# CrystalSixone/VLN-MAGIC

Hardware: AMD Instinct MI355X
Metric: trajectory-steps/sec (whole node), MAGIC-S R2R pretrain (higher is better)
Workload: dtype bf16

## Files before the change

### vln-magic_amd/csrc/encbwd.hip

```cpp
#include "enc_common.hpp"
#include <cstdlib>
#include <cstring>


template <typename Hh> struct RbwSegT {
  int M, kt;
  const Hh* dqkv_n; const Hh* WqkvT_n; const Hh* dao_n;
  const Hh* dfo_in; const Hh* dfod_in;
  const Hh* y2; const float* rstd2; const float* g2; const float* b2; float* dg2; float* db2;
  const Hh* z; const Hh* W2T; const Hh* W1T;
  const Hh* y1; const float* rstd1; const float* g1; const float* b1; float* dg1; float* db1;
  const Hh* WoT;
  Hh *dfo, *dfod, *dz, *daod, *dao, *dctx;
  unsigned site_out, site_ao;
  int mode, N, ntile, ldp;
  const Hh* qkv_a; const Hh* P_a; const Hh* o_a; const Hh* dctx_a; const float* dP_init;
  Hh* dqkv_out;
  unsigned site_attn, pad_;
  const float* dist; float* dsprel_w; float* dsprel_b;
};
template <typename Hh> struct RbwParamsT { RbwSegT<Hh> seg[2]; int nseg, blocks0; float p_hidden; int pad1; const unsigned* seed; float p_attn, scale; };
typedef RbwParamsT<bf16> RbwParams; typedef RbwSegT<bf16> RbwSeg;
#define F(f) ABI_VIEW(RbwSeg, magic_rowbwd_seg, f)
F(M) F(kt) F(dqkv_n) F(WqkvT_n) F(dao_n) F(dfo_in) F(dfod_in) F(y2) F(rstd2) F(g2) F(b2) F(dg2) F(db2) F(z) F(W2T) F(W1T) F(y1) F(rstd1) F(g1) F(b1)
F(dg1) F(db1) F(WoT) F(dfo) F(dfod) F(dz) F(daod) F(dao) F(dctx) F(site_out) F(site_ao) F(mode) F(N) F(ntile) F(ldp) F(qkv_a) F(P_a) F(o_a) F(dctx_a)
F(dP_init) F(dqkv_out) F(site_attn) F(pad_) F(dist) F(dsprel_w) F(dsprel_b)
#undef F
#define F(f) ABI_VIEW(RbwParams, magic_rowbwd_params, f)
F(seg) F(nseg) F(blocks0) F(p_hidden) F(pad1) F(seed) F(p_attn) F(scale)
#undef F

__device__ __forceinline__ float dgelu_fast(float x) {
  const float ax = fabsf(x) * 0.70710678118654752f;
  const float t = __builtin_amdgcn_rcpf(1.0f + 0.3275911f * ax);
  const float poly = t * (0.254829592f + t * (-0.284496736f + t * (1.421413741f + t * (-1.453152027f + t * 1.061405429f))));
  const float e = __expf(-ax * ax);
  const float erf_abs = 1.0f - poly * e;
  const float cdf = 0.5f * (1.0f + (x < 0.f ? -erf_abs : erf_abs));
  return cdf + x * 0.39894228040143268f * e;
}

template <typename Hh> __device__ __forceinline__ void load_rows_img(Hh* s, int pitch, const Hh* g, long long ldg, int rows, int cols, int nvalid, int tid) {
  const int cpr = cols / 8;
  for (int id = tid; id < rows * cpr; id += NWAVE * 64) {
    const int r = id / cpr, c = (id % cpr) * 8;
    h16x8<Hh> v;
#pragma unroll
    for (int e = 0; e < 8; ++e) v[e] = (Hh)0.0f;
    if (r < nvalid) v = *(const h16x8<Hh>*)(g + (long long)r * ldg + c);
    *(h16x8<Hh>*)(s + r * pitch + c) = v;
  }
}

template <int NRT, typename Hh>
__device__ __forceinline__ void ln_bwd_rows(f32x4 (&acc)[NRT], const Hh* sY, const float* rstd_g, const float gm, const float bt, float* dgamma,
                                            float* dbeta, float* red, Hh* sSum, Hh* sDense, const int m0, const int M, const DropState& ds,
                                            const int w, const int lane, const int part_blk = -1) {
  constexpr int RB_ROWS = NRT * 16;
  const int g = lane >> 4, c16 = lane & 15, col = w * 16 + c16;
  const float ig = gm != 0.f ? 1.f / gm : 0.f;
  float xh[NRT][4], s1[NRT][4], s2[NRT][4];
  float pg = 0.f, pb = 0.f;
#pragma unroll
  for (int i = 0; i < NRT; ++i)
#pragma unroll
    for (int r = 0; r < 4; ++r) {
      const int rr = i * 16 + 4 * g + r;
      const bool live = m0 + rr < M;
      const float v = live ? acc[i][r] : 0.f;
      const float x = live ? (to_f(sY[rr * XS + col]) - bt) * ig : 0.f;
      pg += v * x; pb += v;
      const float ga = v * gm;
      acc[i][r] = ga; xh[i][r] = x;
      s1[i][r] = row16_sum(ga); s2[i][r] = row16_sum(ga * x);
    }
  if (dgamma) {
    pg += __shfl_xor(pg, 16, 64); pg += __shfl_xor(pg, 32, 64);
    pb += __shfl_xor(pb, 16, 64); pb += __shfl_xor(pb, 32, 64);
    if (g == 0) {
      if (part_blk >= 0) { dgamma[(long long)part_blk * EH + col] = pg; dbeta[(long long)part_blk * EH + col] = pb; }
      else { atomicAdd(dgamma + col, pg); atomicAdd(dbeta + col, pb); }
    }
  }
  if (c16 == 0) {
#pragma unroll
    for (int i = 0; i < NRT; ++i)
#pragma unroll
      for (int r = 0; r < 4; ++r) { red[w * RB_ROWS + i * 16 + 4 * g + r] = s1[i][r]; red[(NWAVE + w) * RB_ROWS + i * 16 + 4 * g + r] = s2[i][r]; }
  }
  __syncthreads();
#pragma unroll
  for (int i = 0; i < NRT; ++i)
#pragma unroll
    for (int r = 0; r < 4; ++r) {
      const int rr = i * 16 + 4 * g + r;
      float t1 = 0.f, t2 = 0.f;
#pragma unroll
      for (int ww = 0; ww < NWAVE; ++ww) { t1 += red[ww * RB_ROWS + rr]; t2 += red[(NWAVE + ww) * RB_ROWS + rr]; }
      const float m1 = t1 * (1.0f / EH), m2 = t2 * (1.0f / EH);
      const float rs = (m0 + rr < M) ? rstd_g[m0 + rr] : 0.f;
      const float d = rs * (acc[i][r] - m1 - xh[i][r] * m2);
      sSum[rr * XS + col] = from_f<Hh>(d);
      sDense[rr * XS + col] = from_f<Hh>(ds.on ? d * drop_mul(ds, (unsigned)((m0 + rr) * EH + col)) : d);
    }
}

#ifdef RBW_TIMING
__device__ long long rbw_ticks[32];
#define RBW_MARK(i) do { if (blockIdx.x == 0 && threadIdx.x == 0) rbw_ticks[i] = wall_clock64(); } while (0)
#else
#define RBW_MARK(i)
#endif
#define AT_DS 72
#define AT_PS 104
#define AT_ROWS 96
static inline size_t attn_stage_lds() { return (size_t)(3 * AT_ROWS * AT_DS + 3 * 16 * AT_PS) * 2 + AT_ROWS * sizeof(float); }
template <typename Hh, bool DIST>
__device__ __forceinline__ void attn_tile_stage(const RbwSegT<Hh>& sg, const RbwParamsT<Hh>& p, const int b, const int ti, const int nv,
                                                Hh* sDq, unsigned char* scratch, const int tid) {
  typedef h16x4<Hh> v4;
  const int lane = tid & 63, w = __builtin_amdgcn_readfirstlane(tid >> 6), g = lane >> 4, c16 = lane & 15;
  const int N = sg.N, NT = sg.ntile, NK32 = (N + 31) / 32 * 32, ldp = sg.ldp;
  Hh* sQ = (Hh*)scratch;
  Hh* sK = sQ + AT_ROWS * AT_DS;
  Hh* sdO = sK + AT_ROWS * AT_DS;
  Hh* sdS = sdO + AT_ROWS * AT_DS;
  Hh* sdST = sdS + 16 * AT_PS;
  Hh* sPT = sdST + 16 * AT_PS;
  float* sRs = (float*)(sPT + 16 * AT_PS);
  const long long row0 = (long long)b * N;
  DropDesc dd;
  dd.seed = p.seed; dd.site = sg.site_attn; dd.p = p.p_attn;
  const DropState ds = drop_init(dd);
  h16x8<Hh> zero8;
#pragma unroll
  for (int e = 0; e < 8; ++e) zero8[e] = (Hh)0.0f;
  for (int id = tid; id < 3 * 16 * AT_PS / 8; id += NWAVE * 64) *(h16x8<Hh>*)(sdS + id * 8) = zero8;
  constexpr int RIT = (AT_ROWS * 8 + NWAVE * 64 - 1) / (NWAVE * 64);
  static_assert(RIT == 2, "image-row load mapping");
  h16x8<Hh> rq[RIT], rk[RIT], ro[RIT], rO[RIT];
  auto img_issue = [&](const int h) {
#pragma unroll
    for (int it = 0; it < RIT; ++it) {
      const int id = tid + it * NWAVE * 64, r = id >> 3, c = (id & 7) * 8;
      rq[it] = zero8; rk[it] = zero8; ro[it] = zero8; rO[it] = zero8;
      if (r < N) {
        const Hh* base = sg.qkv_a + (row0 + r) * (3 * EH) + h * EHD + c;
        rq[it] = *(const h16x8<Hh>*)base;
        rk[it] = *(const h16x8<Hh>*)(base + EH);
        ro[it] = *(const h16x8<Hh>*)(sg.dctx_a + (row0 + r) * EH + h * EHD + c);
        rO[it] = *(const h16x8<Hh>*)(sg.o_a + (row0 + r) * EH + h * EHD + c);
      }
    }
  };
  auto img_store = [&](const int h) {
#pragma unroll
    for (int it = 0; it < RIT; ++it) {
      const int id = tid + it * NWAVE * 64, r = id >> 3, c = (id & 7) * 8;
      if (r < NK32) {
        *(h16x8<Hh>*)(sQ + r * AT_DS + c) = rq[it];
        *(h16x8<Hh>*)(sK + r * AT_DS + c) = rk[it];
        *(h16x8<Hh>*)(sdO + r * AT_DS + c) = ro[it];
      }
      float s = 0.f;
#pragma unroll
      for (int e = 0; e < 8; ++e) s += to_f(ro[it][e]) * to_f(rO[it][e]);
      if (DIST && sg.dP_init && r < N) {
        const long long prow = ((long long)b * ENH + h) * N + r;
        for (int c8 = (id & 7) * 8; c8 < ldp; c8 += 64) {
          const h16x8<Hh> pv = *(const h16x8<Hh>*)(sg.P_a + prow * ldp + c8);
          const f32x4 i0 = *(const f32x4*)(sg.dP_init + prow * ldp + c8), i1 = *(const f32x4*)(sg.dP_init + prow * ldp + c8 + 4);
#pragma unroll
          for (int e = 0; e < 8; ++e) {
            const int key = c8 + e;
            if (key < N) {
              const float m = ds.on ? drop_mul(ds, (unsigned)(prow * N + key)) : 1.f;
              s += to_f(pv[e]) * m * (e < 4 ? i0[e & 3] : i1[e & 3]);
            }
          }
        }
      }
      s += dpp_mov<DPP_QUAD_XOR1>(s);
      s += dpp_mov<DPP_QUAD_XOR2>(s);
      s += dpp_mov<DPP_ROW_HALF_MIRROR>(s);
      if ((id & 7) == 0 && r < NK32) sRs[r] = s;
    }
  };
  constexpr int AJ = (2 * (AT_ROWS / 16) + NWAVE - 1) / NWAVE;
  h16x8<Hh> av[AJ][EHD / 32];
  v4 ap[AJ];
  f32x4 ai[DIST ? AJ : 1];
  auto vp_issue = [&](const int h) {
#pragma unroll
    for (int jj = 0; jj < AJ; ++jj) {
      const int job = w + NWAVE * jj;
      const bool asq = job < NT;
      const int t = asq ? job : job - NT;
      const int ktile = asq ? t : ti, qtile = asq ? ti : t;
      const int vkey = ktile * 16 + c16, q = qtile * 16 + c16, key0 = ktile * 16 + 4 * g;
      const long long prow = ((long long)b * ENH + h) * N + q;
#pragma unroll
      for (int ks = 0; ks < EHD / 32; ++ks) {
        av[jj][ks] = zero8;
        if (job < 2 * NT && vkey < N) av[jj][ks] = *(const h16x8<Hh>*)(sg.qkv_a + (row0 + vkey) * (3 * EH) + 2 * EH + h * EHD + ks * 32 + 8 * g);
      }
#pragma unroll
      for (int r = 0; r < 4; ++r) ap[jj][r] = (Hh)0.0f;
      if constexpr (DIST) ai[jj] = (f32x4){0.f, 0.f, 0.f, 0.f};
      if (job < 2 * NT && q < N) {
        if (key0 < ldp) ap[jj] = *(const v4*)(sg.P_a + prow * ldp + key0);
        if constexpr (DIST) {
          if (sg.dP_init && key0 < N) ai[jj] = *(const f32x4*)(sg.dP_init + prow * ldp + key0);
        }
      }
    }
  };
  float a0 = 0.f, a1 = 0.f;
  RBW_MARK(16);
  img_issue(0);
  vp_issue(0);
  for (int h = 0; h < ENH; ++h) {
    img_store(h);
    __syncthreads();
    RBW_MARK(17 + 3 * h);
    if (h + 1 < ENH) img_issue(h + 1);
#pragma unroll
    for (int jj = 0; jj < AJ; ++jj) {
      const int job = w + NWAVE * jj;
      if (job < 2 * NT) {
        const bool asq = job < NT;
        const int t = asq ? job : job - NT;
        const int ktile = asq ? t : ti, qtile = asq ? ti : t;
        f32x4 acc = (f32x4){0.f, 0.f, 0.f, 0.f};
#pragma unroll
        for (int ks = 0; ks < EHD / 32; ++ks) acc = mfma16(av[jj][ks], frag_kc(sdO, AT_DS, qtile * 16, ks * 32, lane), acc);
        const int q = qtile * 16 + c16, key0 = ktile * 16 + 4 * g;
        const bool qok = q < N;
        const long long prow = ((long long)b * ENH + h) * N + q;
        const float rsq = sRs[q];
        v4 o4, pm4;
#pragma unroll
        for (int r = 0; r < 4; ++r) {
          const int key = key0 + r;
          const bool ok = qok && key < N;
          float d = acc[r];
          if constexpr (DIST) d += ok ? ai[jj][r] : 0.f;
          const float pp = to_f(ap[jj][r]);
          float pm = pp;
          if (ds.on) {
            const float m = ok ? drop_mul(ds, (unsigned)(prow * N + key)) : 0.f;
            d *= m; pm = pp * m;
          }
          const float dsu = pp * (d - rsq);
          o4[r] = from_f<Hh>(dsu * p.scale);
          pm4[r] = from_f<Hh>(pm);
          if constexpr (DIST) {
            if (sg.dist && asq && ok) { a0 += dsu * sg.dist[((long long)b * N + q) * N + key]; a1 += dsu; }
          }
        }
        if (asq) *(v4*)(sdS + c16 * AT_PS + key0) = o4;
        else {
#pragma unroll
          for (int r = 0; r < 4; ++r) { sdST[(4 * g + r) * AT_PS + q] = o4[r]; sPT[(4 * g + r) * AT_PS + q] = pm4[r]; }
        }
      }
    }
    if (h + 1 < ENH) vp_issue(h + 1);
    __syncthreads();
    RBW_MARK(18 + 3 * h);
    for (int job = w; job < 12; job += NWAVE) {
      const int prod = job >> 2, jd = job & 3;
      const Hh* A = prod == 0 ? sdS : (prod == 1 ? sdST : sPT);
      const Hh* Bm = prod == 0 ? sK : (prod == 1 ? sQ : sdO);
      f32x4 acc = (f32x4){0.f, 0.f, 0.f, 0.f};
      for (int ks = 0; ks < NK32 / 32; ++ks) acc = mfma16(frag_kc(A, AT_PS, 0, ks * 32, lane), frag_oc(Bm, AT_DS, jd * 16, ks * 32, lane), acc);
      const int col = prod * EH + h * EHD + jd * 16 + c16;
#pragma unroll
      for (int r = 0; r < 4; ++r) sDq[(4 * g + r) * QS + col] = from_f<Hh>(acc[r]);
    }
    __syncthreads();
    RBW_MARK(19 + 3 * h);
  }
  copy_out(sDq, QS, sg.dqkv_out + (row0 + ti * 16) * (3 * EH), 3 * EH, nv, 3 * EH, tid);
  if (DIST && sg.dist) {
    a0 = wave_sum(a0); a1 = wave_sum(a1);
    if (lane == 0) { sRs[w] = a0; sRs[NWAVE + w] = a1; }
    __syncthreads();
    if (tid == 0) {
      float s0 = 0.f, s1 = 0.f;
#pragma unroll
      for (int i = 0; i < NWAVE; ++i) { s0 += sRs[i]; s1 += sRs[NWAVE + i]; }
      atomicAdd(sg.dsprel_w, s0);
      atomicAdd(sg.dsprel_b, s1);
    }
    __syncthreads();
  }
  RBW_MARK(23);
}

template <int NRT, typename Hh, int ATT = 0>
__device__ __forceinline__ void rowbwd_body(const RbwParamsT<Hh>& p, unsigned char* rb_smem) {
  constexpr int RB_ROWS = NRT * 16;
  constexpr bool DEEP = NRT >= 4;
  static_assert(!ATT || NRT == 1, "the attention stage works on 16-row tiles of one sample");
  int blk = blockIdx.x, sidx = 0;
  if (blk >= p.blocks0) { blk -= p.blocks0; sidx = 1; }
  const RbwSegT<Hh>& sg = p.seg[sidx];
  const int mode = ATT ? sg.mode : 0;
  Hh* sZ = (Hh*)rb_smem;
  Hh* sY2 = sZ + RB_ROWS * GS;
  Hh* sR = sY2 + RB_ROWS * XS;
  Hh* sFo = sR + RB_ROWS * XS;
  Hh* sD = sFo + RB_ROWS * XS;
  Hh* sY1 = sD + RB_ROWS * XS;
  Hh* sAo = sR;
  float* red = (float*)(sY1 + RB_ROWS * XS);
  const int tid = threadIdx.x, lane = tid & 63, w = __builtin_amdgcn_readfirstlane(tid >> 6), g = lane >> 4, c16 = lane & 15;
  const int M = sg.M;
  int m0 = blk * RB_ROWS, nv = min(RB_ROWS, M - m0);
  if (mode) { const int b = blk / sg.ntile, ti = blk - b * sg.ntile; m0 = b * sg.N + ti * 16; nv = min(16, sg.N - ti * 16); }
  const int colw = w * 16 + c16;
  const bool tail = mode ? true : sg.dqkv_n != nullptr;
  const bool shortm = sg.z == nullptr;
  const int kt = mode ? 12 : sg.kt, ldq = kt * 32;
  DropDesc dd;
  dd.seed = p.seed; dd.p = p.p_hidden;
  RBW_MARK(0);
  if (mode) {
    const int b = blk / sg.ntile;
    attn_tile_stage<Hh, ATT == 2>(sg, p, b, blk - b * sg.ntile, nv, sZ, rb_smem + (size_t)RB_ROWS * GS * sizeof(Hh), tid);
  }
  h16x8<Hh> wq[12];
  if (tail) {
#pragma unroll
    for (int ks = 0; ks < (DEEP ? 12 : 4); ++ks)
      if (ks < kt) wq[ks] = gfrag(sg.WqkvT_n, ldq, w * 16, ks * 32, lane);
  }
  h16x8<Hh> w2[4][4];
  const float gm2 = mode == 2 ? 0.f : sg.g2[colw], bt2 = mode == 2 ? 0.f : sg.b2[colw];
  const float gm1 = shortm ? 0.f : sg.g1[colw], bt1 = shortm ? 0.f : sg.b1[colw];
  if (mode) ;
  else if (tail) load_rows_img(sZ, QS, sg.dqkv_n + (long long)m0 * ldq, ldq, RB_ROWS, ldq, nv, tid);
  else load_rows_img(sZ, GS, sg.z + (long long)m0 * EI, EI, RB_ROWS, EI, nv, tid);
  if (!shortm) load_rows_img(sY1, XS, sg.y1 + (long long)m0 * EH, EH, RB_ROWS, EH, nv, tid);
  if (tail) {
    if (mode != 2) load_rows_img(sY2, XS, sg.y2 + (long long)m0 * EH, EH, RB_ROWS, EH, nv, tid);
    load_rows_img(sR, XS, sg.dao_n + (long long)m0 * EH, EH, RB_ROWS, EH, nv, tid);
  } else {
    load_rows_img(sFo, XS, sg.dfo_in + (long long)m0 * EH, EH, RB_ROWS, EH, nv, tid);
    load_rows_img(sD, XS, sg.dfod_in + (long long)m0 * EH, EH, RB_ROWS, EH, nv, tid);
  }
  __syncthreads();
  RBW_MARK(1);
  if (tail) {
    f32x4 acc[NRT];
#pragma unroll
    for (int i = 0; i < NRT; ++i) acc[i] = (f32x4){0.f, 0.f, 0.f, 0.f};
#pragma unroll
    for (int ch = 0; ch < 3; ++ch) {
      if (4 * ch >= kt) break;
      if (!DEEP && ch < 2 && 4 * ch + 4 < kt) {
#pragma unroll
        for (int ks = 4 * ch + 4; ks < 4 * ch + 8; ++ks) wq[ks] = gfrag(sg.WqkvT_n, ldq, w * 16, ks * 32, lane);
      }
#pragma unroll
      for (int ks = 4 * ch; ks < 4 * ch + 4; ++ks) {
#pragma unroll
        for (int i = 0; i < NRT; ++i) acc[i] = mfma16(frag_kc(sZ, QS, i * 16, ks * 32, lane), wq[ks], acc[i]);
      }
      KSTEP_FENCE();
    }
    RBW_MARK(2);
    if (mode == 2) {
#pragma unroll
      for (int i = 0; i < NRT; ++i)
#pragma unroll
        for (int r = 0; r < 4; ++r) {
          const int rr = i * 16 + 4 * g + r;
          sFo[rr * XS + colw] = from_f<Hh>(acc[i][r] + to_f(sR[rr * XS + colw]));
        }
      __syncthreads();
      copy_out(sFo, XS, sg.dfo + (long long)m0 * EH, EH, nv, EH, tid);
      return;
    }
    constexpr int ZIT = RB_ROWS * (EI / 8) / (NWAVE * 64);
    h16x8<Hh> zr[ZIT];
#pragma unroll
    for (int it = 0; it < ZIT; ++it) {
      const int id = tid + it * NWAVE * 64, r = id / (EI / 8), c = (id % (EI / 8)) * 8;
#pragma unroll
      for (int e = 0; e < 8; ++e) zr[it][e] = (Hh)0.0f;
      if (r < nv && !shortm) zr[it] = *(const h16x8<Hh>*)(sg.z + (long long)(m0 + r) * EI + c);
    }
#pragma unroll
    for (int i = 0; i < NRT; ++i)
#pragma unroll
      for (int r = 0; r < 4; ++r) acc[i][r] += to_f(sR[(i * 16 + 4 * g + r) * XS + colw]);
    dd.site = sg.site_out;
    const DropState ds = drop_init(dd);
    ln_bwd_rows<NRT>(acc, sY2, sg.rstd2, gm2, bt2, sg.dg2, sg.db2, red, sFo, sD, m0, m0 + nv, ds, w, lane, p.pad1 ? blk : -1);
#pragma unroll
    for (int it = 0; it < ZIT; ++it) {
      const int id = tid + it * NWAVE * 64, r = id / (EI / 8), c = (id % (EI / 8)) * 8;
      *(h16x8<Hh>*)(sZ + r * GS + c) = zr[it];
    }
    __syncthreads();
    RBW_MARK(3);
    copy_out(sFo, XS, sg.dfo + (long long)m0 * EH, EH, nv, EH, tid);
    copy_out(sD, XS, sg.dfod + (long long)m0 * EH, EH, nv, EH, tid);
  }
  RBW_MARK(4);
  h16x8<Hh> wo[4];
  if (shortm) {
#pragma unroll
    for (int ks = 0; ks < 4; ++ks) wo[ks] = gfrag(sg.WoT, EH, w * 16, ks * 32, lane);
  } else {
  h16x8<Hh> w1[16];
  {
    f32x4 acc[NRT][4];
#pragma unroll
    for (int i = 0; i < NRT; ++i)
#pragma unroll
      for (int ct = 0; ct < 4; ++ct) acc[i][ct] = (f32x4){0.f, 0.f, 0.f, 0.f};
#pragma unroll
    for (int ct = 0; ct < 4; ++ct) w2[ct][0] = gfrag(sg.W2T, EH, (4 * w + ct) * 16, 0, lane);
#pragma unroll
    for (int ks = 0; ks < 4; ++ks) {
      if (ks < 3) {
#pragma unroll
        for (int ct = 0; ct < 4; ++ct) w2[ct][ks + 1] = gfrag(sg.W2T, EH, (4 * w + ct) * 16, (ks + 1) * 32, lane);
      }
#pragma unroll
      for (int i = 0; i < NRT; ++i) {
        const h16x8<Hh> a = frag_kc(sD, XS, i * 16, ks * 32, lane);
#pragma unroll
        for (int ct = 0; ct < 4; ++ct) acc[i][ct] = mfma16(a, w2[ct][ks], acc[i][ct]);
      }
      KSTEP_FENCE();
    }
#pragma unroll
    for (int ks = 0; ks < (DEEP ? 8 : 4); ++ks) w1[ks] = gfrag(sg.W1T, EI, w * 16, ks * 32, lane);
#pragma unroll
    for (int ct = 0; ct < 4; ++ct) {
      const int col = (4 * w + ct) * 16 + c16;
#pragma unroll
      for (int i = 0; i < NRT; ++i)
#pragma unroll
        for (int r = 0; r < 4; ++r) {
          const int rr = i * 16 + 4 * g + r;
          Hh* e = sZ + rr * GS + col;
          *e = from_f<Hh>(acc[i][ct][r] * dgelu_fast(to_f(*e)));
        }
    }
  }
  __syncthreads();
  RBW_MARK(5);
  copy_out(sZ, GS, sg.dz + (long long)m0 * EI, EI, nv, EI, tid);
  RBW_MARK(6);
  {
    f32x4 acc[NRT];
#pragma unroll
    for (int i = 0; i < NRT; ++i) acc[i] = (f32x4){0.f, 0.f, 0.f, 0.f};
    constexpr int CHK = DEEP ? 8 : 4;
#pragma unroll
    for (int ch = 0; ch < 16 / CHK; ++ch) {
      if (ch + 1 < 16 / CHK) {
#pragma unroll
        for (int ks = CHK * (ch + 1); ks < CHK * (ch + 2); ++ks) w1[ks] = gfrag(sg.W1T, EI, w * 16, ks * 32, lane);
      } else {
#pragma unroll
        for (int ks = 0; ks < 4; ++ks) wo[ks] = gfrag(sg.WoT, EH, w * 16, ks * 32, lane);
      }
#pragma unroll
      for (int ks = CHK * ch; ks < CHK * (ch + 1); ++ks) {
#pragma unroll
        for (int i = 0; i < NRT; ++i) acc[i] = mfma16(frag_kc(sZ, GS, i * 16, ks * 32, lane), w1[ks], acc[i]);
        if ((ks & 3) == 3) KSTEP_FENCE();
      }
    }
#pragma unroll
    for (int i = 0; i < NRT; ++i)
#pragma unroll
      for (int r = 0; r < 4; ++r) acc[i][r] += to_f(sFo[(i * 16 + 4 * g + r) * XS + colw]);
    RBW_MARK(7);
    dd.site = sg.site_ao;
    const DropState ds = drop_init(dd);
    ln_bwd_rows<NRT>(acc, sY1, sg.rstd1, gm1, bt1, sg.dg1, sg.db1, red, sAo, sD, m0, m0 + nv, ds, w, lane, p.pad1 ? blk : -1);
  }
  __syncthreads();
  RBW_MARK(8);
  copy_out(sAo, XS, sg.dao + (long long)m0 * EH, EH, nv, EH, tid);
  copy_out(sD, XS, sg.daod + (long long)m0 * EH, EH, nv, EH, tid);
  }
  RBW_MARK(9);
  {
    f32x4 acc[NRT];
#pragma unroll
    for (int i = 0; i < NRT; ++i) acc[i] = (f32x4){0.f, 0.f, 0.f, 0.f};
#pragma unroll
    for (int ks = 0; ks < 4; ++ks)
#pragma unroll
      for (int i = 0; i < NRT; ++i) acc[i] = mfma16(frag_kc(sD, XS, i * 16, ks * 32, lane), wo[ks], acc[i]);
#pragma unroll
    for (int i = 0; i < NRT; ++i)
#pragma unroll
      for (int r = 0; r < 4; ++r) sY2[(i * 16 + 4 * g + r) * XS + colw] = from_f<Hh>(acc[i][r]);
  }
  __syncthreads();
  RBW_MARK(10);
  copy_out(sY2, XS, sg.dctx + (long long)m0 * EH, EH, nv, EH, tid);
  RBW_MARK(11);
}

template <typename Hh> __global__ __launch_bounds__(512, 4) void rowbwd16_kernel(RbwParamsT<Hh> p) {
  extern __shared__ __attribute__((aligned(16))) unsigned char rb_smem[];
  rowbwd_body<1>(p, rb_smem);
}
template <typename Hh> __global__ __launch_bounds__(512, 4) void rowbwd32_kernel(RbwParamsT<Hh> p) {
  extern __shared__ __attribute__((aligned(16))) unsigned char rb_smem[];
  rowbwd_body<2>(p, rb_smem);
}
template <typename Hh> __global__ __launch_bounds__(512, 2) void rowbwd64_kernel(RbwParamsT<Hh> p) {
  extern __shared__ __attribute__((aligned(16))) unsigned char rb_smem[];
  rowbwd_body<4>(p, rb_smem);
}
template <typename Hh> __global__ __launch_bounds__(512, 4) void rowbwd16a_kernel(RbwParamsT<Hh> p) {
  extern __shared__ __attribute__((aligned(16))) unsigned char rb_smem[];
  rowbwd_body<1, Hh, 1>(p, rb_smem);
}
template <typename Hh> __global__ __launch_bounds__(512, 4) void rowbwd16ad_kernel(RbwParamsT<Hh> p) {
  extern __shared__ __attribute__((aligned(16))) unsigned char rb_smem[];
  rowbwd_body<1, Hh, 2>(p, rb_smem);
}
static size_t rbw_lds_bytes(int rows) { return (size_t)(rows * GS + 5 * rows * XS) * 2 + (size_t)2 * NWAVE * rows * sizeof(float); }
static int rbw_rows_env() {
  static int r = -1;
  if (r < 0) { const char* e = getenv("MAGIC_RBW_ROWS"); const int v = e ? atoi(e) : 0; r = (v == 16 || v == 32 || v == 64) ? v : 0; }
  return r;
}
static int rbw_ncu() {
  static int n = 0;
  if (!n) { hipDeviceProp_t pr; int d = 0; (void)hipGetDevice(&d); n = (hipGetDeviceProperties(&pr, d) == hipSuccess) ? pr.multiProcessorCount : 256; }
  return n;
}

extern "C" int magic_rowbwd_rows(long long total_rows) { return rbw_rows_env() ? rbw_rows_env() : (total_rows <= 16ll * rbw_ncu() ? 16 : 32); }

__global__ __launch_bounds__(1024) void colsum_add_kernel(ColsumJobs js, int H) {
  __shared__ float red[1024];
  colsum_body(js, blockIdx.x, H, red);
}
extern "C" int magic_colsum_add(int H, int n, const float* const* parts, float* const* dsts, const int* nblks, void* stream) {
  if (n <= 0 || n > CSJ_MAX || !parts || !dsts || !nblks || H <= 0 || H > 1024 || (1024 % H)) return MAGIC_ERR_ARG;
  ColsumJobs js;
  js.n = n;
  for (int i = 0; i < n; ++i) {
    if (!parts[i] || !dsts[i] || nblks[i] <= 0) return MAGIC_ERR_ARG;
    js.part[i] = parts[i]; js.dst[i] = dsts[i]; js.nblk[i] = nblks[i];
  }
  hipLaunchKernelGGL(colsum_add_kernel, dim3(n), dim3(1024), 0, (hipStream_t)stream, js, H);
  return launch_status();
}

extern "C" int magic_rowbwd_attn_supported(int dtype, int H, int I, int nh, int N) { return dtype_is16(dtype) && H == EH && I == EI && nh == ENH && N > 0 && N <= AT_ROWS; }
extern "C" int magic_rowbwd_supported(int dtype, int H, int I) { return dtype_is16(dtype) && H == EH && I == EI; }
extern "C" int magic_rowbwd_params_bytes() { return (int)sizeof(RbwParams); }

extern "C" int magic_rowbwd(int dtype, const void* params, int nbytes, void* stream) {
  if (!params || nbytes != (int)sizeof(RbwParams) || !dtype_is16(dtype)) return MAGIC_ERR_ARG;
  RbwParams p;
  memcpy(&p, params, sizeof(p));
  if (p.nseg < 1 || p.nseg > 2 || !drop_args_ok(p.seed, p.p_hidden)) return MAGIC_ERR_ARG;
  int blocks = 0;
  long long total_rows = 0;
  bool att = false;
  for (int s = 0; s < p.nseg; ++s) { total_rows += p.seg[s].M > 0 ? p.seg[s].M : 0; att = att || p.seg[s].mode != 0; }
  const int rows = att ? 16 : (rbw_rows_env() ? rbw_rows_env() : (total_rows <= 16ll * rbw_ncu() ? 16 : 32));
  if (att && !drop_args_ok(p.seed, p.p_attn)) return MAGIC_ERR_ARG;
  for (int s = 0; s < 2; ++s) {
    RbwSeg& sg = p.seg[s];
    if (s >= p.nseg) { sg.M = 0; sg.mode = 0; continue; }
    if (sg.M <= 0 || (long long)sg.M * EI > 0x7FFFFFFFll) return MAGIC_ERR_ARG;
    if (sg.mode) {
      if (sg.mode != 1 && sg.mode != 2) return MAGIC_ERR_ARG;
      if (sg.N <= 0 || sg.N > AT_ROWS || sg.M % sg.N || sg.ldp < sg.N || sg.ldp % 8 || sg.ntile != (sg.N + 15) / 16) return MAGIC_ERR_ARG;
      const void* need[] = {sg.qkv_a, sg.P_a, sg.o_a, sg.dctx_a, sg.dqkv_out, sg.WqkvT_n, sg.dao_n, sg.dfo};
      for (const void* q : need)
        if (!q || ((uintptr_t)q & 15)) return MAGIC_ERR_ARG;
      if (((uintptr_t)sg.dP_init & 15) || (long long)(sg.M / sg.N) * ENH * sg.N * sg.N > 0xFFFFFFFFll) return MAGIC_ERR_ARG;
      if ((sg.dist == nullptr) != (sg.dsprel_w == nullptr) || (sg.dist == nullptr) != (sg.dsprel_b == nullptr)) return MAGIC_ERR_ARG;
      if (sg.mode == 2) {
        const int nb2 = (sg.M / sg.N) * sg.ntile;
        if (s == 0) p.blocks0 = nb2;
        blocks += nb2;
        continue;
      }
      if (!sg.z || !sg.dfod) return MAGIC_ERR_ARG;
    }
    const void* req[] = {sg.y2, sg.rstd2, sg.g2, sg.b2, sg.WoT, sg.dctx};
    for (const void* q : req)
      if (!q) return MAGIC_ERR_ARG;
    if (sg.z) {
      const void* full[] = {sg.W2T, sg.W1T, sg.y1, sg.rstd1, sg.g1, sg.b1, sg.dz, sg.daod, sg.dao};
      for (const void* q : full)
        if (!q) return MAGIC_ERR_ARG;
    } else if (!sg.dqkv_n) return MAGIC_ERR_ARG;
    if (sg.mode) ;
    else if (sg.dqkv_n) { if (!sg.WqkvT_n || !sg.dao_n || !sg.dfo || !sg.dfod || (sg.kt != 0 && sg.kt != 4 && sg.kt != 12)) return MAGIC_ERR_ARG; }
    else if (!sg.dfo_in || !sg.dfod_in) return MAGIC_ERR_ARG;
    if ((sg.dg2 == nullptr) != (sg.db2 == nullptr) || (sg.dg1 == nullptr) != (sg.db1 == nullptr)) return MAGIC_ERR_ARG;
    const void* al[] = {sg.dqkv_n, sg.WqkvT_n, sg.dao_n, sg.dfo_in, sg.dfod_in, sg.y2, sg.z, sg.W2T, sg.W1T, sg.y1, sg.WoT, sg.dfo, sg.dfod, sg.dz, sg.daod, sg.dao, sg.dctx};
    for (const void* q : al)
      if ((uintptr_t)q & 15) return MAGIC_ERR_ARG;
    const int nb = sg.mode ? (sg.M / sg.N) * sg.ntile : (sg.M + rows - 1) / rows;
    if (s == 0) p.blocks0 = nb;
    blocks += nb;
  }
  if (att) {
    const size_t rest = rbw_lds_bytes(16) - (size_t)16 * GS * 2;
    const size_t shm = (size_t)16 * GS * 2 + (attn_stage_lds() > rest ? attn_stage_lds() : rest);
    static bool attr_a = false;
    if (!attr_a) {
      (void)hipFuncSetAttribute((const void*)rowbwd16a_kernel<bf16>, hipFuncAttributeMaxDynamicSharedMemorySize, (int)shm);
      (void)hipFuncSetAttribute((const void*)rowbwd16a_kernel<f16>, hipFuncAttributeMaxDynamicSharedMemorySize, (int)shm);
      (void)hipFuncSetAttribute((const void*)rowbwd16ad_kernel<bf16>, hipFuncAttributeMaxDynamicSharedMemorySize, (int)shm);
      (void)hipFuncSetAttribute((const void*)rowbwd16ad_kernel<f16>, hipFuncAttributeMaxDynamicSharedMemorySize, (int)shm);
      attr_a = true;
    }
    const bool with_dist = (p.seg[0].mode && (p.seg[0].dist || p.seg[0].dP_init)) || (p.nseg > 1 && p.seg[1].mode && (p.seg[1].dist || p.seg[1].dP_init));
    if (with_dist) DISPATCH_H(dtype, hipLaunchKernelGGL(rowbwd16ad_kernel<TY>, dim3(blocks), dim3(512), shm, (hipStream_t)stream, view_as<RbwParamsT<TY>>(p)));
    else DISPATCH_H(dtype, hipLaunchKernelGGL(rowbwd16a_kernel<TY>, dim3(blocks), dim3(512), shm, (hipStream_t)stream, view_as<RbwParamsT<TY>>(p)));
    return launch_status();
  }
  const size_t shm = rbw_lds_bytes(rows);
  static bool attr_set = false;
  if (!attr_set) {
#define RBW_ATTR(TY)                                                                                                              \
    (void)hipFuncSetAttribute((const void*)rowbwd16_kernel<TY>, hipFuncAttributeMaxDynamicSharedMemorySize, (int)rbw_lds_bytes(16)); \
    (void)hipFuncSetAttribute((const void*)rowbwd32_kernel<TY>, hipFuncAttributeMaxDynamicSharedMemorySize, (int)rbw_lds_bytes(32)); \
    (void)hipFuncSetAttribute((const void*)rowbwd64_kernel<TY>, hipFuncAttributeMaxDynamicSharedMemorySize, (int)rbw_lds_bytes(64))
    RBW_ATTR(bf16); RBW_ATTR(f16);
#undef RBW_ATTR
    attr_set = true;
  }
  DISPATCH_H(dtype,
    const RbwParamsT<TY> pt = view_as<RbwParamsT<TY>>(p);
    if (rows == 16) hipLaunchKernelGGL(rowbwd16_kernel<TY>, dim3(blocks), dim3(512), shm, (hipStream_t)stream, pt);
    else if (rows == 32) hipLaunchKernelGGL(rowbwd32_kernel<TY>, dim3(blocks), dim3(512), shm, (hipStream_t)stream, pt);
    else hipLaunchKernelGGL(rowbwd64_kernel<TY>, dim3(blocks), dim3(512), shm, (hipStream_t)stream, pt));
  return launch_status();
}

typedef __attribute__((ext_vector_type(8))) unsigned short u16x8;
#define TSP_MAX 160
struct TSpans { long long off[TSP_MAX]; int rows[TSP_MAX]; int cols[TSP_MAX]; int tile0[TSP_MAX + 1]; int n; };
__global__ __launch_bounds__(256) void transpose_spans_kernel(const unsigned short* __restrict__ src, unsigned short* __restrict__ dst, TSpans t) {
  __shared__ unsigned short tile[32][34];
  const int id = blockIdx.x;
  int s = 0;
  for (int i = 1; i < t.n; ++i) s += (id >= t.tile0[i]) ? 1 : 0;
  const int local = id - t.tile0[s], R = t.rows[s], C = t.cols[s];
  const int tc = (C + 31) / 32, r0 = (local / tc) * 32, c0 = (local % tc) * 32;
  const unsigned short* a = src + t.off[s];
  unsigned short* b = dst + t.off[s];
  const int tx = threadIdx.x & 31, ty = threadIdx.x >> 5;
  for (int j = ty; j < 32; j += 8)
    if (r0 + j < R && c0 + tx < C) tile[j][tx] = a[(long long)(r0 + j) * C + c0 + tx];
  __syncthreads();
  for (int j = ty; j < 32; j += 8)
    if (c0 + j < C && r0 + tx < R) b[(long long)(c0 + j) * R + r0 + tx] = tile[tx][j];
}
__global__ __launch_bounds__(256) void transpose_spans64_kernel(const unsigned short* __restrict__ src, unsigned short* __restrict__ dst, TSpans t) {
  __shared__ unsigned short tile[64][72];
  const int id = blockIdx.x;
  int s = 0;
  for (int i = 1; i < t.n; ++i) s += (id >= t.tile0[i]) ? 1 : 0;
  const int local = id - t.tile0[s], R = t.rows[s], C = t.cols[s];
  const int tc = C / 64, r0 = (local / tc) * 64, c0 = (local % tc) * 64;
  const unsigned short* a = src + t.off[s];
  unsigned short* b = dst + t.off[s];
#pragma unroll
  for (int it = 0; it < 2; ++it) {
    const int ch = threadIdx.x + it * 256, r = ch >> 3, c = (ch & 7) * 8;
    *(u16x8*)&tile[r][c] = *(const u16x8*)(a + (long long)(r0 + r) * C + c0 + c);
  }
  __syncthreads();
#pragma unroll
  for (int it = 0; it < 2; ++it) {
    const int ch = threadIdx.x + it * 256, cc = ch >> 3, rr = (ch & 7) * 8;
    u16x8 v;
#pragma unroll
    for (int e = 0; e < 8; ++e) v[e] = tile[rr + e][cc];
    *(u16x8*)(b + (long long)(c0 + cc) * R + r0 + rr) = v;
  }
}
extern "C" int magic_transpose_spans(const void* src, void* dst, int n, const long long* offs, const int* rows, const int* cols, void* stream) {
  if (!src || !dst || n < 0 || (n && (!offs || !rows || !cols))) return MAGIC_ERR_ARG;
  bool all64 = !((uintptr_t)src & 15) && !((uintptr_t)dst & 15);
  for (int i = 0; i < n && all64; ++i) all64 = rows[i] > 0 && cols[i] > 0 && rows[i] % 64 == 0 && cols[i] % 64 == 0 && offs[i] % 8 == 0;
  const int ts = all64 ? 64 : 32;
  for (int base = 0; base < n; base += TSP_MAX) {
    TSpans t;
    t.n = n - base < TSP_MAX ? n - base : TSP_MAX;
    int tiles = 0;
    for (int i = 0; i < t.n; ++i) {
      if (rows[base + i] <= 0 || cols[base + i] <= 0) return MAGIC_ERR_ARG;
      t.off[i] = offs[base + i]; t.rows[i] = rows[base + i]; t.cols[i] = cols[base + i];
      t.tile0[i] = tiles;
      tiles += ((rows[base + i] + ts - 1) / ts) * ((cols[base + i] + ts - 1) / ts);
    }
    t.tile0[t.n] = tiles;
    if (all64) hipLaunchKernelGGL(transpose_spans64_kernel, dim3(tiles), dim3(256), 0, (hipStream_t)stream, (const unsigned short*)src, (unsigned short*)dst, t);
    else hipLaunchKernelGGL(transpose_spans_kernel, dim3(tiles), dim3(256), 0, (hipStream_t)stream, (const unsigned short*)src, (unsigned short*)dst, t);
  }
  return launch_status();
}
```

Before: 197,300.

## Prefetch tail-stage rows and Wqkv fragments during attention backward, dedupe diagonal tile job

The attention backward tile stage now takes a callback. During the last head it issues global loads for the dao/y2/y1 rows and the first four WqkvT fragments that the following row-backward tail needs, so those loads overlap the final head's MFMA work instead of running after it. The diagonal tile (ktile==qtile==ti) is handled once, writing both the dS and transposed buffers, which removes one redundant job. Address arithmetic is rewritten as 32-bit offsets behind opaque asm barriers to keep indexing in scalar and small vector registers. The cost is extra register pressure from holding the prefetched fragments, plus reliance on a hard-coded layout for the WqkvT fragments (kt==12).

```diff
diff --git a/vln-magic_amd/csrc/encbwd.hip b/vln-magic_amd/csrc/encbwd.hip
--- a/vln-magic_amd/csrc/encbwd.hip
+++ b/vln-magic_amd/csrc/encbwd.hip
@@ -114,10 +114,17 @@
 #define AT_DS 72
 #define AT_PS 104
 #define AT_ROWS 96
+__device__ __forceinline__ int at_opaque(int v) { asm volatile("" : "+s"(v)); return v; }
+__device__ __forceinline__ int at_opaque_v(int v) { asm volatile("" : "+v"(v)); return v; }
+template <typename V, typename T> __device__ __forceinline__ V at_ld(const T* base, const unsigned off) {
+  unsigned o = off * (unsigned)sizeof(T);
+  asm volatile("" : "+v"(o));
+  return *(const V*)((const char*)base + (size_t)o);
+}
 static inline size_t attn_stage_lds() { return (size_t)(3 * AT_ROWS * AT_DS + 3 * 16 * AT_PS) * 2 + AT_ROWS * sizeof(float); }
-template <typename Hh, bool DIST>
+template <typename Hh, bool DIST, typename Pre>
 __device__ __forceinline__ void attn_tile_stage(const RbwSegT<Hh>& sg, const RbwParamsT<Hh>& p, const int b, const int ti, const int nv,
-                                                Hh* sDq, unsigned char* scratch, const int tid) {
+                                                Hh* sDq, unsigned char* scratch, const int tid, Pre&& chain_prefetch) {
   typedef h16x4<Hh> v4;
   const int lane = tid & 63, w = __builtin_amdgcn_readfirstlane(tid >> 6), g = lane >> 4, c16 = lane & 15;
   const int N = sg.N, NT = sg.ntile, NK32 = (N + 31) / 32 * 32, ldp = sg.ldp;
@@ -136,27 +143,38 @@
 #pragma unroll
   for (int e = 0; e < 8; ++e) zero8[e] = (Hh)0.0f;
   for (int id = tid; id < 3 * 16 * AT_PS / 8; id += NWAVE * 64) *(h16x8<Hh>*)(sdS + id * 8) = zero8;
+  const Hh* const qkv_s = sg.qkv_a + row0 * (3 * EH);
+  const Hh* const dO_s = sg.dctx_a + row0 * EH;
+  const Hh* const O_s = sg.o_a + row0 * EH;
+  const float* const dist_s = DIST && sg.dist ? sg.dist + row0 * N : nullptr;
+  const bool seeded = DIST && sg.dP_init != nullptr;
   constexpr int RIT = (AT_ROWS * 8 + NWAVE * 64 - 1) / (NWAVE * 64);
   static_assert(RIT == 2, "image-row load mapping");
   h16x8<Hh> rq[RIT], rk[RIT], ro[RIT], rO[RIT];
-  auto img_issue = [&](const int h) {
+  auto img_issue = [&](const int h_) {
+    const int h = at_opaque(h_), t_ = at_opaque_v(tid);
 #pragma unroll
     for (int it = 0; it < RIT; ++it) {
-      const int id = tid + it * NWAVE * 64, r = id >> 3, c = (id & 7) * 8;
+      const int id = t_ + it * NWAVE * 64, r = id >> 3, c = (id & 7) * 8;
       rq[it] = zero8; rk[it] = zero8; ro[it] = zero8; rO[it] = zero8;
       if (r < N) {
-        const Hh* base = sg.qkv_a + (row0 + r) * (3 * EH) + h * EHD + c;
-        rq[it] = *(const h16x8<Hh>*)base;
-        rk[it] = *(const h16x8<Hh>*)(base + EH);
-        ro[it] = *(const h16x8<Hh>*)(sg.dctx_a + (row0 + r) * EH + h * EHD + c);
-        rO[it] = *(const h16x8<Hh>*)(sg.o_a + (row0 + r) * EH + h * EHD + c);
+        const unsigned oq = (unsigned)(r * (3 * EH) + c), oo = (unsigned)(r * EH + c);
+        rq[it] = at_ld<h16x8<Hh>>(qkv_s + h * EHD, oq);
+        rk[it] = at_ld<h16x8<Hh>>(qkv_s + h * EHD + EH, oq);
+        ro[it] = at_ld<h16x8<Hh>>(dO_s + h * EHD, oo);
+        rO[it] = at_ld<h16x8<Hh>>(O_s + h * EHD, oo);
       }
     }
   };
-  auto img_store = [&](const int h) {
+  auto img_store = [&](const int h_) {
+    const int h = at_opaque(h_), t_ = at_opaque_v(tid);
+    const long long prow0 = ((long long)b * ENH + h) * N;
+    const Hh* const P_h = sg.P_a + prow0 * ldp;
+    const float* const I_h = seeded ? sg.dP_init + prow0 * ldp : nullptr;
+    const unsigned didx0 = (unsigned)(prow0 * N);
 #pragma unroll
     for (int it = 0; it < RIT; ++it) {
-      const int id = tid + it * NWAVE * 64, r = id >> 3, c = (id & 7) * 8;
+      const int id = t_ + it * NWAVE * 64, r = id >> 3, c = (id & 7) * 8;
       if (r < NK32) {
         *(h16x8<Hh>*)(sQ + r * AT_DS + c) = rq[it];
         *(h16x8<Hh>*)(sK + r * AT_DS + c) = rk[it];
@@ -165,16 +183,17 @@
       float s = 0.f;
 #pragma unroll
       for (int e = 0; e < 8; ++e) s += to_f(ro[it][e]) * to_f(rO[it][e]);
-      if (DIST && sg.dP_init && r < N) {
-        const long long prow = ((long long)b * ENH + h) * N + r;
-        for (int c8 = (id & 7) * 8; c8 < ldp; c8 += 64) {
-          const h16x8<Hh> pv = *(const h16x8<Hh>*)(sg.P_a + prow * ldp + c8);
-          const f32x4 i0 = *(const f32x4*)(sg.dP_init + prow * ldp + c8), i1 = *(const f32x4*)(sg.dP_init + prow * ldp + c8 + 4);
+      if (seeded && r < N) {
+#pragma unroll 1
+        for (int c8 = c; c8 < ldp; c8 += 64) {
+          const unsigned op = (unsigned)(r * ldp + c8);
+          const h16x8<Hh> pv = at_ld<h16x8<Hh>>(P_h, op);
+          const f32x4 i0 = at_ld<f32x4>(I_h, op), i1 = at_ld<f32x4>(I_h, op + 4);
 #pragma unroll
           for (int e = 0; e < 8; ++e) {
             const int key = c8 + e;
             if (key < N) {
-              const float m = ds.on ? drop_mul(ds, (unsigned)(prow * N + key)) : 1.f;
+              const float m = ds.on ? drop_mul(ds, didx0 + (unsigned)(r * N + key)) : 1.f;
               s += to_f(pv[e]) * m * (e < 4 ? i0[e & 3] : i1[e & 3]);
             }
           }
@@ -186,31 +205,41 @@
       if ((id & 7) == 0 && r < NK32) sRs[r] = s;
     }
   };
-  constexpr int AJ = (2 * (AT_ROWS / 16) + NWAVE - 1) / NWAVE;
+  constexpr int AJ = (2 * (AT_ROWS / 16) - 1 + NWAVE - 1) / NWAVE;
+  const int NJ = 2 * NT - 1;
   h16x8<Hh> av[AJ][EHD / 32];
   v4 ap[AJ];
   f32x4 ai[DIST ? AJ : 1];
-  auto vp_issue = [&](const int h) {
+  auto job_tiles = [&](const int job, bool& asq, int& ktile, int& qtile) {
+    asq = job < NT;
+    const int t = asq ? job : job - NT + (job - NT >= ti ? 1 : 0);
+    ktile = asq ? t : ti; qtile = asq ? ti : t;
+  };
+  auto vp_issue = [&](const int h_) {
+    const int h = at_opaque(h_), l_ = at_opaque_v(lane), g = l_ >> 4, c16 = l_ & 15;
+    const long long prow0 = ((long long)b * ENH + h) * N;
+    const Hh* const P_h = sg.P_a + prow0 * ldp;
+    const float* const I_h = seeded ? sg.dP_init + prow0 * ldp : nullptr;
+    const Hh* const V_h = qkv_s + 2 * EH + h * EHD;
 #pragma unroll
     for (int jj = 0; jj < AJ; ++jj) {
       const int job = w + NWAVE * jj;
-      const bool asq = job < NT;
-      const int t = asq ? job : job - NT;
-      const int ktile = asq ? t : ti, qtile = asq ? ti : t;
+      bool asq; int ktile, qtile;
+      job_tiles(job, asq, ktile, qtile);
       const int vkey = ktile * 16 + c16, q = qtile * 16 + c16, key0 = ktile * 16 + 4 * g;
-      const long long prow = ((long long)b * ENH + h) * N + q;
 #pragma unroll
       for (int ks = 0; ks < EHD / 32; ++ks) {
         av[jj][ks] = zero8;
-        if (job < 2 * NT && vkey < N) av[jj][ks] = *(const h16x8<Hh>*)(sg.qkv_a + (row0 + vkey) * (3 * EH) + 2 * EH + h * EHD + ks * 32 + 8 * g);
+        if (job < NJ && vkey < N) av[jj][ks] = at_ld<h16x8<Hh>>(V_h, (unsigned)(vkey * (3 * EH) + ks * 32 + 8 * g));
       }
 #pragma unroll
       for (int r = 0; r < 4; ++r) ap[jj][r] = (Hh)0.0f;
       if constexpr (DIST) ai[jj] = (f32x4){0.f, 0.f, 0.f, 0.f};
-      if (job < 2 * NT && q < N) {
-        if (key0 < ldp) ap[jj] = *(const v4*)(sg.P_a + prow * ldp + key0);
+      if (job < NJ && q < N) {
+        const unsigned op = (unsigned)(q * ldp + key0);
+        if (key0 < ldp) ap[jj] = at_ld<v4>(P_h, op);
         if constexpr (DIST) {
-          if (sg.dP_init && key0 < N) ai[jj] = *(const f32x4*)(sg.dP_init + prow * ldp + key0);
+          if (seeded && key0 < N) ai[jj] = at_ld<f32x4>(I_h, op);
         }
       }
     }
@@ -224,19 +253,20 @@
     __syncthreads();
     RBW_MARK(17 + 3 * h);
     if (h + 1 < ENH) img_issue(h + 1);
+    const unsigned didx_h = (unsigned)(((long long)b * ENH + h) * N * N);
+    const int lane = at_opaque_v(tid & 63), g = lane >> 4, c16 = lane & 15;
 #pragma unroll
     for (int jj = 0; jj < AJ; ++jj) {
       const int job = w + NWAVE * jj;
-      if (job < 2 * NT) {
-        const bool asq = job < NT;
-        const int t = asq ? job : job - NT;
-        const int ktile = asq ? t : ti, qtile = asq ? ti : t;
+      if (job < NJ) {
+        bool asq; int ktile, qtile;
+        job_tiles(job, asq, ktile, qtile);
+        const bool both = asq && ktile == ti;
         f32x4 acc = (f32x4){0.f, 0.f, 0.f, 0.f};
 #pragma unroll
         for (int ks = 0; ks < EHD / 32; ++ks) acc = mfma16(av[jj][ks], frag_kc(sdO, AT_DS, qtile * 16, ks * 32, lane), acc);
         const int q = qtile * 16 + c16, key0 = ktile * 16 + 4 * g;
         const bool qok = q < N;
-        const long long prow = ((long long)b * ENH + h) * N + q;
         const float rsq = sRs[q];
         v4 o4, pm4;
 #pragma unroll
@@ -248,18 +278,18 @@
           const float pp = to_f(ap[jj][r]);
           float pm = pp;
           if (ds.on) {
-            const float m = ok ? drop_mul(ds, (unsigned)(prow * N + key)) : 0.f;
+            const float m = ok ? drop_mul(ds, didx_h + (unsigned)(q * N + key)) : 0.f;
             d *= m; pm = pp * m;
           }
           const float dsu = pp * (d - rsq);
           o4[r] = from_f<Hh>(dsu * p.scale);
           pm4[r] = from_f<Hh>(pm);
           if constexpr (DIST) {
-            if (sg.dist && asq && ok) { a0 += dsu * sg.dist[((long long)b * N + q) * N + key]; a1 += dsu; }
+            if (dist_s && asq && ok) { a0 += dsu * at_ld<float>(dist_s, (unsigned)(q * N + key)); a1 += dsu; }
           }
         }
         if (asq) *(v4*)(sdS + c16 * AT_PS + key0) = o4;
-        else {
+        if (!asq || both) {
 #pragma unroll
           for (int r = 0; r < 4; ++r) { sdST[(4 * g + r) * AT_PS + q] = o4[r]; sPT[(4 * g + r) * AT_PS + q] = pm4[r]; }
         }
@@ -268,6 +298,7 @@
     if (h + 1 < ENH) vp_issue(h + 1);
     __syncthreads();
     RBW_MARK(18 + 3 * h);
+    if (h == ENH - 1) chain_prefetch();
     for (int job = w; job < 12; job += NWAVE) {
       const int prod = job >> 2, jd = job & 3;
       const Hh* A = prod == 0 ? sdS : (prod == 1 ? sdST : sPT);
@@ -298,6 +329,12 @@
   RBW_MARK(23);
 }
 
+template <typename Hh> __device__ __forceinline__ const RbwSegT<Hh>& seg_at(const RbwParamsT<Hh>& p, const int sidx) {
+  unsigned off = (unsigned)sidx * (unsigned)sizeof(RbwSegT<Hh>);
+  asm volatile("" : "+s"(off));
+  return *(const RbwSegT<Hh>*)((const char*)&p.seg[0] + off);
+}
+
 template <int NRT, typename Hh, int ATT = 0>
 __device__ __forceinline__ void rowbwd_body(const RbwParamsT<Hh>& p, unsigned char* rb_smem) {
   constexpr int RB_ROWS = NRT * 16;
@@ -305,8 +342,8 @@
   static_assert(!ATT || NRT == 1, "the attention stage works on 16-row tiles of one sample");
   int blk = blockIdx.x, sidx = 0;
   if (blk >= p.blocks0) { blk -= p.blocks0; sidx = 1; }
-  const RbwSegT<Hh>& sg = p.seg[sidx];
-  const int mode = ATT ? sg.mode : 0;
+  const RbwSegT<Hh>& sg0 = ATT ? seg_at(p, sidx) : p.seg[sidx];
+  const int mode = ATT ? sg0.mode : 0;
   Hh* sZ = (Hh*)rb_smem;
   Hh* sY2 = sZ + RB_ROWS * GS;
   Hh* sR = sY2 + RB_ROWS * XS;
@@ -316,39 +353,62 @@
   Hh* sAo = sR;
   float* red = (float*)(sY1 + RB_ROWS * XS);
   const int tid = threadIdx.x, lane = tid & 63, w = __builtin_amdgcn_readfirstlane(tid >> 6), g = lane >> 4, c16 = lane & 15;
-  const int M = sg.M;
+  const int M = sg0.M;
   int m0 = blk * RB_ROWS, nv = min(RB_ROWS, M - m0);
-  if (mode) { const int b = blk / sg.ntile, ti = blk - b * sg.ntile; m0 = b * sg.N + ti * 16; nv = min(16, sg.N - ti * 16); }
+  if (mode) { const int b = blk / sg0.ntile, ti = blk - b * sg0.ntile; m0 = b * sg0.N + ti * 16; nv = min(16, sg0.N - ti * 16); }
   const int colw = w * 16 + c16;
+  RBW_MARK(0);
+  h16x8<Hh> pre[ATT ? 3 : 1], wqp[ATT ? 4 : 1];
+  const int pr = tid >> 4, pc = (tid & 15) * 8;
+  if (mode) {
+    const int b = blk / sg0.ntile;
+    attn_tile_stage<Hh, ATT == 2>(sg0, p, b, blk - b * sg0.ntile, nv, sZ, rb_smem + (size_t)RB_ROWS * GS * sizeof(Hh), tid, [&]() {
+#pragma unroll
+      for (int i = 0; i < 3; ++i)
+#pragma unroll
+        for (int e = 0; e < 8; ++e) pre[i][e] = (Hh)0.0f;
+      const int t_ = at_opaque_v(tid), r_ = t_ >> 4;
+      if (t_ < 256 && r_ < nv) {
+        const long long o0 = (long long)m0 * EH;
+        const unsigned o = (unsigned)(r_ * EH + (t_ & 15) * 8);
+        pre[0] = at_ld<h16x8<Hh>>(sg0.dao_n + o0, o);
+        if (mode != 2) { pre[1] = at_ld<h16x8<Hh>>(sg0.y2 + o0, o); pre[2] = at_ld<h16x8<Hh>>(sg0.y1 + o0, o); }
+      }
+#pragma unroll
+      for (int ks = 0; ks < 4; ++ks) wqp[ks] = at_ld<h16x8<Hh>>(sg0.WqkvT_n + (long long)(w * (12 * 64 * 8) + ks * 64 * 8), (unsigned)((t_ & 63) * 8));
+    });
+  }
+  const RbwSegT<Hh>& sg = ATT ? seg_at(p, sidx) : sg0;
   const bool tail = mode ? true : sg.dqkv_n != nullptr;
   const bool shortm = sg.z == nullptr;
   const int kt = mode ? 12 : sg.kt, ldq = kt * 32;
   DropDesc dd;
   dd.seed = p.seed; dd.p = p.p_hidden;
-  RBW_MARK(0);
-  if (mode) {
-    const int b = blk / sg.ntile;
-    attn_tile_stage<Hh, ATT == 2>(sg, p, b, blk - b * sg.ntile, nv, sZ, rb_smem + (size_t)RB_ROWS * GS * sizeof(Hh), tid);
-  }
   h16x8<Hh> wq[12];
   if (tail) {
 #pragma unroll
     for (int ks = 0; ks < (DEEP ? 12 : 4); ++ks)
-      if (ks < kt) wq[ks] = gfrag(sg.WqkvT_n, ldq, w * 16, ks * 32, lane);
+      if (ks < kt) wq[ks] = (ATT && mode) ? wqp[ATT ? ks : 0] : gfrag(sg.WqkvT_n, ldq, w * 16, ks * 32, lane);
   }
   h16x8<Hh> w2[4][4];
   const float gm2 = mode == 2 ? 0.f : sg.g2[colw], bt2 = mode == 2 ? 0.f : sg.b2[colw];
   const float gm1 = shortm ? 0.f : sg.g1[colw], bt1 = shortm ? 0.f : sg.b1[colw];
-  if (mode) ;
-  else if (tail) load_rows_img(sZ, QS, sg.dqkv_n + (long long)m0 * ldq, ldq, RB_ROWS, ldq, nv, tid);
-  else load_rows_img(sZ, GS, sg.z + (long long)m0 * EI, EI, RB_ROWS, EI, nv, tid);
-  if (!shortm) load_rows_img(sY1, XS, sg.y1 + (long long)m0 * EH, EH, RB_ROWS, EH, nv, tid);
-  if (tail) {
-    if (mode != 2) load_rows_img(sY2, XS, sg.y2 + (long long)m0 * EH, EH, RB_ROWS, EH, nv, tid);
-    load_rows_img(sR, XS, sg.dao_n + (long long)m0 * EH, EH, RB_ROWS, EH, nv, tid);
+  if (mode) {
+    if (tid < 256) {
+      *(h16x8<Hh>*)(sR + pr * XS + pc) = pre[0];
+      if (mode != 2) { *(h16x8<Hh>*)(sY2 + pr * XS + pc) = pre[1]; *(h16x8<Hh>*)(sY1 + pr * XS + pc) = pre[2]; }
+    }
   } else {
-    load_rows_img(sFo, XS, sg.dfo_in + (long long)m0 * EH, EH, RB_ROWS, EH, nv, tid);
-    load_rows_img(sD, XS, sg.dfod_in + (long long)m0 * EH, EH, RB_ROWS, EH, nv, tid);
+    if (tail) load_rows_img(sZ, QS, sg.dqkv_n + (long long)m0 * ldq, ldq, RB_ROWS, ldq, nv, tid);
+    else load_rows_img(sZ, GS, sg.z + (long long)m0 * EI, EI, RB_ROWS, EI, nv, tid);
+    if (!shortm) load_rows_img(sY1, XS, sg.y1 + (long long)m0 * EH, EH, RB_ROWS, EH, nv, tid);
+    if (tail) {
+      if (mode != 2) load_rows_img(sY2, XS, sg.y2 + (long long)m0 * EH, EH, RB_ROWS, EH, nv, tid);
+      load_rows_img(sR, XS, sg.dao_n + (long long)m0 * EH, EH, RB_ROWS, EH, nv, tid);
+    } else {
+      load_rows_img(sFo, XS, sg.dfo_in + (long long)m0 * EH, EH, RB_ROWS, EH, nv, tid);
+      load_rows_img(sD, XS, sg.dfod_in + (long long)m0 * EH, EH, RB_ROWS, EH, nv, tid);
+    }
   }
   __syncthreads();
   RBW_MARK(1);
```

Result: no change. 198,800, median of 6 (+0.7%).
